# josehu07/summerset

Measured on AMD Instinct MI355X. Metric: committed_slots_per_sec, higher is better.
Workload: dtype u64; 1 GPU; MultiPaxos lock-step, 65536 groups/GPU x 5 replicas, S=32 new slots/group/tick, heartbeat every 4 ticks, 10% ack loss (<= 2 lost per slot), 59.53% of the groups per 4286 ticks with a leader timeout (9; groups_per_gpu=65536, replicas=5, slots_per_tick=32, window=512, layout=colocated

## Files before the change

### include/summerset_hip.h

```cpp
#ifndef SUMMERSET_HIP_H
#define SUMMERSET_HIP_H

#include <stddef.h>
#include <stdint.h>

#ifdef __cplusplus
extern "C" {
#endif

#define SMR_OK 0
#define SMR_ERR_ARG (-1)
#define SMR_ERR_DEVICE (-2)
#define SMR_ERR_STATE (-3)

#define SMR_NO_REPLICA 0xFFu
#define SMR_MAX_REPLICAS 8

enum { SMR_ST_NULL = 0, SMR_ST_PREPARING = 1, SMR_ST_ACCEPTING = 2, SMR_ST_COMMITTED = 3, SMR_ST_EXECUTED = 4 };

#define SMR_CTL_IDENTITY 0x00FAC688u

const char *smr_last_error(void);
int smr_device_count(void);
uint32_t smr_abi_version(void);
// ... 126 lines not shown

int smr_mp_ack_matrix(smr_mp_cluster *c, uint8_t rep, uint8_t **ack_dev, uint64_t *n_bytes);

typedef struct {
    uint32_t group, slot;
    uint64_t ballot;
    uint32_t peer;
    uint32_t reserved;
} smr_mp_ack;
int smr_mp_deliver_acks(smr_mp_cluster *c, uint8_t rep, const smr_mp_ack *acks_dev, uint64_t n, uint64_t *dropped_dev,
                        void *stream);
int smr_mp_deliver_acks_conn(smr_mp_cluster *c, uint8_t rep, const void *acks12_dev, uint64_t ack_cap, const uint64_t *conn_off_dev,
                             const uint32_t *conn_group_dev, const uint8_t *conn_peer_dev, const uint32_t *cnt_dev, uint32_t n_conn,
                             uint64_t *dropped_dev, void *stream);
int smr_mp_collect_acks(smr_mp_cluster *c, uint8_t rep, smr_mp_ack *out_dev, uint64_t cap, uint64_t *n_dev, void *stream);
int smr_mp_clear_acks(smr_mp_cluster *c, uint8_t rep, void *stream);

int smr_mp_debug_arena_view(smr_mp_cluster *c, void **base_dev, uint64_t *n_bytes);

int smr_mp_read_group_state(smr_mp_cluster *c, uint32_t group, uint8_t rep, smr_mp_group_state *out);

typedef struct {
    uint8_t *leader; uint64_t *bal_prep_sent, *bal_prepared, *bal_max_seen;
    uint32_t *start_slot, *log_len, *accept_bar, *commit_bar, *exec_bar, *snap_bar;
    uint32_t *peer_exec_bar;
    uint64_t *s_bal; uint8_t *s_status; uint32_t *s_reqs; uint64_t *s_vbal; uint32_t *s_vreqs;
    uint8_t *s_flags, *s_acks, *s_packs; uint64_t *s_pmax; uint32_t *s_ltrig, *s_lendp;
    uint8_t *s_src; uint32_t *s_rtrig, *s_rendp;
    uint8_t *overflow;
} smr_mp_dump_bufs;
int smr_mp_dump(smr_mp_cluster *c, uint8_t rep, const smr_mp_dump_bufs *host_bufs);
int smr_mp_dump_range(smr_mp_cluster *c, uint8_t rep, uint32_t g0, uint32_t n, const smr_mp_dump_bufs *host_bufs);

typedef struct smr_mp_snapshot smr_mp_snapshot;
typedef struct {
    uint64_t bytes;
    uint64_t n_slots, n_outbox;
    uint32_t n_groups, max_live, max_outbox;
    uint8_t population, commit_extra, live_mask, reserved;
} smr_mp_snapshot_info;
int smr_mp_snapshot_create(const smr_mp_cluster *like, smr_mp_snapshot **out);
void smr_mp_snapshot_destroy(smr_mp_snapshot *s);
int smr_mp_save_state(smr_mp_cluster *c, smr_mp_snapshot *s, void *stream);
int smr_mp_load_state(smr_mp_cluster *c, const smr_mp_snapshot *s, void *stream);
int smr_mp_snapshot_info_get(const smr_mp_snapshot *s, smr_mp_snapshot_info *out);
int64_t smr_mp_snapshot_export(const smr_mp_snapshot *s, uint8_t *host, uint64_t cap);
int smr_mp_snapshot_import(smr_mp_snapshot *s, const uint8_t *host, uint64_t len);

int smr_mp_counters(smr_mp_cluster *c, uint8_t rep, uint64_t out[3]);

int smr_mp_debug_generic_units(smr_mp_cluster *c, uint8_t rep, uint64_t *out);

int smr_mp_debug_folded_batches(smr_mp_cluster *c, uint8_t rep, uint64_t *out);

int smr_mp_straggler_stats(smr_mp_cluster *c, uint64_t out[2]);

int smr_mp_debug_stamps(smr_mp_cluster *c, uint64_t *out64);

int smr_mp_poll_commits(smr_mp_cluster *c, uint8_t rep, uint32_t *groups_host, uint32_t *slots_host,
                        uint64_t cap, uint64_t *n_out);

int smr_mp_profile_enable(smr_mp_cluster *c, int on);
int smr_mp_profile_read(smr_mp_cluster *c, int which, double *total_ms, uint64_t *launches);

typedef struct smr_raft_leader smr_raft_leader;

typedef struct {
    uint32_t n_groups;
    uint8_t population;
    uint8_t leader_id;
    uint8_t commit_extra;
    uint8_t reserved0;
    uint32_t window;
    uint64_t term;
} smr_raft_cfg;

int smr_raft_leader_create(const smr_raft_cfg *cfg, smr_raft_leader **out);
void smr_raft_leader_destroy(smr_raft_leader *l);
int smr_raft_leader_append(smr_raft_leader *l, const uint32_t *n_new_dev, void *stream);
int smr_raft_leader_handle_replies(smr_raft_leader *l, const uint64_t *reply_term_dev,
                                   const uint32_t *end_slot_dev, const uint64_t *conflict_term_dev,
                                   const uint32_t *conflict_slot_dev, const uint8_t *flags_dev,
                                   const uint32_t *order_dev, void *stream);
typedef struct {
    const uint32_t *n_new;
    const uint64_t *reply_term;
    const uint32_t *end_slot;
    const uint64_t *conflict_term;
    const uint32_t *conflict_slot;
    const uint8_t *flags;
    const uint32_t *order;
} smr_raft_tick;
int smr_raft_leader_run_ticks(smr_raft_leader *l, const smr_raft_tick *ticks, uint32_t n_ticks, void *stream);
typedef struct {
    uint8_t *role; uint64_t *curr_term; uint32_t *log_len, *last_commit, *last_snap;
    uint32_t *next_slot, *try_next_slot, *match_slot;
    uint64_t *entry_term;
    uint8_t *leader; uint32_t *start_slot;
} smr_raft_dump_bufs;
int smr_raft_leader_dump(smr_raft_leader *l, const smr_raft_dump_bufs *host_bufs);
int smr_raft_leader_total_commits(smr_raft_leader *l, uint64_t *out);

int smr_raft_craft_enable(smr_raft_leader *l, uint8_t fault_tolerance, uint8_t repeat_threshold);
int smr_raft_craft_bcast_heartbeats(smr_raft_leader *l, uint8_t *hb_flags_dev, uint32_t *prev_slot_dev, uint64_t *prev_term_dev,
                                    uint32_t *leader_commit_dev, uint32_t *last_snap_dev, void *stream);
int smr_raft_craft_switch_assignment_mode(smr_raft_leader *l, const uint8_t *to_full_dev, void *stream);
// ... 651 lines not shown
```

### summerset_amd/_lib.py

```python
import ctypes as C
import os

_HERE = os.path.dirname(os.path.abspath(__file__))
LIB_PATH = os.path.join(_HERE, "libsummerset_hip.so")

SMR_OK, SMR_ERR_ARG, SMR_ERR_DEVICE, SMR_ERR_STATE = 0, -1, -2, -3
SMR_NO_REPLICA = 0xFF
SMR_MAX_REPLICAS = 8
SMR_CTL_IDENTITY = 0x00FAC688


class SummersetError(RuntimeError):

    def __init__(self, code, msg):
        super().__init__("[%d] %s" % (code, msg))
        self.code = code
        self.msg = msg


class MpCfg(C.Structure):
    _fields_ = [("n_groups", C.c_uint32), ("population", C.c_uint8), ("commit_extra", C.c_uint8),
                ("straggler_ticks", C.c_uint8), ("reserved1", C.c_uint8), ("window", C.c_uint32),
                ("win_reserve", C.c_uint32), ("outbox_cap", C.c_uint32), ("commit_list_cap", C.c_uint32)]

# ... 190 lines not shown
    _fields_ = [("kind", C.c_uint8), ("has_voted", C.c_uint8), ("n_items", C.c_uint32), ("slot", C.c_uint64),
                ("ballot", C.c_uint64), ("trigger_slot", C.c_uint64), ("endprep_slot", C.c_uint64), ("voted_ballot", C.c_uint64),
                ("commit_bar", C.c_uint64), ("exec_bar", C.c_uint64), ("snap_bar", C.c_uint64)]


SYMBOLS = [
    ("smr_last_error", C.c_char_p, []),
    ("smr_device_count", _i, []),
    ("smr_abi_version", _u32, []),
    ("smr_rs_matrix", _i, [_i, _i, _vp]),
    ("smr_rs_shard_len", _u64, [_u64, _i]),
    ("smr_rs_encode", _i, [_vp, _u64, _u64, _u64, _i, _i, _vp, _u64, _u64, _vp]),
    ("smr_rs_encode_lut", _i, [_vp, _u64, _u64, _u64, _i, _i, _vp, _u64, _u64, _vp]),
    ("smr_rs_from_data_encode", _i, [_vp, _u64, _u64, _u64, _i, _i, _vp, _u64, _vp]),
    ("smr_rs_from_data_encode_fanout", _i, [_vp, _u64, _u64, _u64, _i, _i, _vp, _u64, _vp, _u64, _u64, _u32, _vp]),
    ("smr_rs_from_data_encode_stores", _i, [_vp, _u64, _u64, _u64, _i, _i, _vp, _u64, _u64, _vp]),
    ("smr_rs_from_data_encode_scatter", _i, [_vp, _u64, _u64, _u64, _i, _i, _vp, _u64, _vp, _u64, _vp]),
    ("smr_rs_reconstruct", _i, [_vp, _u64, _u64, _u64, _u64, _i, _i, _u32, _i, _vp]),
    ("smr_rs_verify", _i, [_vp, _u64, _u64, _u64, _u64, _i, _i, _vp, _vp]),
    ("smr_mp_cluster_create", _i, [C.POINTER(MpCfg), C.POINTER(_vp)]),
    ("smr_mp_cluster_destroy", None, [_vp]),
    ("smr_mp_preset_leader", _i, [_vp, _u8]),
    ("smr_mp_tick", _i, [_vp, _vp, _vp, _vp, _vp, _vp, _u32, _vp, _i, _vp]),
    ("smr_mp_run_ticks", _i, [_vp, C.POINTER(MpTickIn), _u32, _vp]),
    ("smr_mp_set_live", _i, [_vp, _u32]),
    ("smr_mp_set_role_rotation", _i, [_vp, _i]),
    ("smr_mp_image_bytes", C.c_int64, [_vp, _i, _u32, _u32]),
    ("smr_mp_image_pack", _i, [_vp, _i, _u8, _u8, _vp, _u64, _u32, _u32, _vp]),
    ("smr_mp_image_unpack", _i, [_vp, _i, _u8, _u8, _vp, _u64, _u32, _u32, _vp]),
    ("smr_mp_image_plan_create", _i, [C.POINTER(MpImageOp), _u32, _u32, _u32, C.POINTER(_vp)]),
    ("smr_mp_image_plan_destroy", None, [_vp]),
    ("smr_mp_image_plan_run", _i, [_vp, _i, _vp]),
    ("smr_mp_round_local", _i, [_vp, _vp, _vp, _vp, _vp, _vp, _u32, _vp]),
    ("smr_mp_round_deliver", _i, [_vp, _vp]),
    ("smr_mp_round_replies", _i, [_vp, _vp, _i, _vp]),
    ("smr_mp_round_heartbeat", _i, [_vp, _vp]),
    ("smr_mp_end_tick", _i, [_vp]),
    ("smr_mp_spread_create", _i, [_vp, _u32, _vp, _vp, _vp]),
    ("smr_mp_spread_destroy", None, [_vp]),
    ("smr_mp_spread_segment", _i, [_vp, _i, _vp, _i, _vp]),
    ("smr_mp_spread_set_concurrent", _i, [_vp, _i]),
    ("smr_mp_spread_abort_tick", _i, [_vp]),
    ("smr_mp_ack_matrix", _i, [_vp, _u8, C.POINTER(_vp), C.POINTER(_u64)]),
    ("smr_mp_deliver_acks", _i, [_vp, _u8, _vp, _u64, _vp, _vp]),
    ("smr_mp_deliver_acks_conn", _i, [_vp, _u8, _vp, _u64, _vp, _vp, _vp, _vp, _u32, _vp, _vp]),
    ("smr_mp_collect_acks", _i, [_vp, _u8, _vp, _u64, _vp, _vp]),
    ("smr_mp_clear_acks", _i, [_vp, _u8, _vp]),
    ("smr_mp_read_group_state", _i, [_vp, _u32, _u8, C.POINTER(MpGroupState)]),
    ("smr_mp_dump", _i, [_vp, _u8, C.POINTER(MpDumpBufs)]),
    ("smr_mp_dump_range", _i, [_vp, C.c_uint8, _u32, _u32, C.POINTER(MpDumpBufs)]),
    ("smr_mp_counters", _i, [_vp, _u8, C.POINTER(_u64 * 3)]),
    ("smr_mp_debug_generic_units", _i, [_vp, _u8, C.POINTER(_u64)]),
    ("smr_mp_debug_folded_batches", _i, [_vp, _u8, C.POINTER(_u64)]),
    ("smr_mp_debug_stamps", _i, [_vp, _vp]),
    ("smr_comm_unique_id", _i, [_vp, _u64]),
    ("smr_comm_init_rank", _i, [_vp, _u64, _u32, _u32, C.POINTER(_vp)]),
    ("smr_comm_destroy", None, [_vp]),
    ("smr_comm_exchange", _i, [_vp, _vp, C.POINTER(_u64), _vp, C.POINTER(_u64), _u32, _vp]),
    ("smr_comm_all_reduce_u64", _i, [_vp, _vp, _u64, _i, _vp]),
    ("smr_comm_info", _i, [_vp, C.POINTER(_u64 * 5)]),
    ("smr_mp_spread_bind_comm", _i, [_vp, _vp, C.POINTER(_vp * 3), C.POINTER(_u64), C.POINTER(_vp * 3), C.POINTER(_u64), _u32]),
    ("smr_mp_spread_tick", _i, [_vp, _vp, _i, _vp]),
    ("smr_mp_straggler_stats", _i, [_vp, C.POINTER(_u64 * 2)]),
    ("smr_mp_poll_commits", _i, [_vp, _u8, _vp, _vp, _u64, C.POINTER(_u64)]),
    ("smr_mp_debug_arena_view", _i, [_vp, C.POINTER(_vp), C.POINTER(_u64)]),
    ("smr_mp_snapshot_create", _i, [_vp, C.POINTER(_vp)]),
    ("smr_mp_snapshot_destroy", None, [_vp]),
    ("smr_mp_save_state", _i, [_vp, _vp, _vp]),
    ("smr_mp_load_state", _i, [_vp, _vp, _vp]),
    ("smr_mp_snapshot_info_get", _i, [_vp, C.POINTER(MpSnapshotInfo)]),
    ("smr_mp_snapshot_export", C.c_int64, [_vp, _vp, _u64]),
    ("smr_mp_snapshot_import", _i, [_vp, _vp, _u64]),
    ("smr_mp_profile_enable", _i, [_vp, _i]),
    ("smr_mp_profile_read", _i, [_vp, _i, C.POINTER(C.c_double), C.POINTER(_u64)]),
    ("smr_raft_leader_create", _i, [C.POINTER(RaftCfg), C.POINTER(_vp)]),
    ("smr_raft_leader_destroy", None, [_vp]),
    ("smr_raft_leader_append", _i, [_vp, _vp, _vp]),
    ("smr_raft_leader_handle_replies", _i, [_vp, _vp, _vp, _vp, _vp, _vp, _vp, _vp]),
    ("smr_raft_leader_handle_wire_replies", _i, [_vp, _vp, _u64, _vp, _vp, _u32, _vp, _vp, _u64, _vp, _vp, _vp, _vp]),
    ("smr_raft_leader_run_ticks", _i, [_vp, _vp, _u32, _vp]),
    ("smr_raft_leader_dump", _i, [_vp, C.POINTER(RaftDumpBufs)]),
    ("smr_raft_leader_total_commits", _i, [_vp, C.POINTER(_u64)]),
    ("smr_raft_replica_preset", _i, [_vp, _u8, _u8, _u64, _u8]),
    ("smr_raft_replica_handle_append_entries", _i, [_vp, C.POINTER(RaftAppendEntries), C.POINTER(RaftAppendReply), _vp]),
    ("smr_raft_replica_become_candidate", _i, [_vp, _vp, _vp, _vp, _vp, _vp, _vp]),
    ("smr_raft_replica_handle_request_vote", _i, [_vp, _vp, _vp, _vp, _vp, _vp, _vp, _vp, _vp]),
    ("smr_raft_replica_handle_vote_replies", _i, [_vp, _vp, _vp, _vp, _vp, _vp, _vp]),
    ("smr_raft_replica_dump_votes", _i, [_vp, _vp, _vp, _vp, _vp]),
    ("smr_raft_leader_append_emit", _i, [_vp, _vp, _vp, _vp]),
    ("smr_raft_leader_gather_entries", _i, [_vp, _vp, C.POINTER(RaftAppendEntries), _vp]),
    ("smr_raft_cluster_replicate", _i, [_vp, _u32, C.POINTER(_vp), C.POINTER(_vp), C.POINTER(RaftAppendEntries), C.POINTER(RaftAppendReply), _vp]),
    ("smr_raft_cluster_tick", _i, [_vp, _vp, _vp, _u32, C.POINTER(_vp), C.POINTER(_vp), C.POINTER(RaftAppendEntries), C.POINTER(RaftAppendReply), _vp, _vp, _vp, _vp, _vp, _vp, _vp]),
    ("smr_raft_craft_enable", _i, [_vp, _u8, _u8]),
    ("smr_raft_craft_bcast_heartbeats", _i, [_vp, _vp, _vp, _vp, _vp, _vp, _vp]),
    ("smr_raft_craft_switch_assignment_mode", _i, [_vp, _vp, _vp]),
    ("smr_raft_craft_assignment", _i, [_vp, _vp, _vp, _vp]),
    ("smr_raft_craft_dump", _i, [_vp, _vp, _vp, _vp, _vp, _vp]),
    ("smr_raft_craft_handle_reconstruct", _i, [_vp, _vp, _vp, _vp, _u32, _vp, _vp, _vp, _vp]),
    ("smr_raft_craft_dump_masks", _i, [_vp, _vp, _vp]),
    ("smr_raft_ring_guard_hits", _i, [_vp, C.POINTER(_u64)]),
    ("smr_raft_snapshot_create", _i, [_vp, C.POINTER(_vp)]),
    ("smr_raft_snapshot_destroy", None, [_vp]),
    ("smr_raft_save_state", _i, [_vp, _vp, _vp]),
    ("smr_raft_load_state", _i, [_vp, _vp, _vp]),
    ("smr_raft_snapshot_info_get", _i, [_vp, C.POINTER(RaftSnapshotInfo)]),
    ("smr_raft_snapshot_export", C.c_int64, [_vp, _vp, _u64]),
# ... 243 lines not shown
```

### summerset_amd/csrc/mp_engine.hip

```cpp
#include <stdlib.h>
#include <string.h>

#include <algorithm>
#include <functional>
#include <vector>

#include "mp_device.h"
#include "smr_common.h"
#include "mp_snapshot.h"

#ifdef SMR_BULK_PRIO
#define SMR_RAISE_PRIO() __builtin_amdgcn_s_setprio(SMR_BULK_PRIO)
#else
#define SMR_RAISE_PRIO() ((void)0)
#endif

namespace smr {

__device__ __forceinline__ void flush_counters(const Lane &L, bool active) {
    unsigned int c[4] = {active ? L.n_commit : 0u, active ? L.n_redirect : 0u, active ? L.n_reject : 0u,
                         active ? L.n_generic : 0u};
    const bool any = (c[0] | c[1] | c[2] | c[3]) != 0;
    for (unsigned long long todo = __ballot(any); todo;) {
        const uint32_t rep = __shfl(L.me, __ffsll((long long)todo) - 1);
// ... 1180 lines not shown
    uint32_t g;
    const bool active = pick_group(P, side, g);
    r4_body(P, par, g, active, pick_replica(P, side, g));
}

#ifndef STRAG_MINW
#define STRAG_MINW 1
#endif
#ifndef STRAG_K
#define STRAG_K 1
#endif
__global__ __launch_bounds__(512, STRAG_MINW) void mp_straggler_tick(const MpParams *__restrict__ Pp, int par, int lpar,
                                                          const uint8_t *__restrict__ timeout_rep,
                                                          const uint8_t *__restrict__ timeout_src,
                                                          const uint8_t *__restrict__ req_target,
                                                          const uint32_t *__restrict__ req_cnt,
                                                          const uint32_t *__restrict__ req_val, uint32_t S,
                                                          const uint32_t *__restrict__ ackctl, int do_heartbeat) {
    const MpParams &P = *Pp;
    const uint32_t w = threadIdx.x >> 6, lane = threadIdx.x & 63;
    uint32_t n = P.slow_n[lpar];
    if (n > P.slow_cap) n = P.slow_cap;
    for (uint32_t idx0 = blockIdx.x; idx0 < n; idx0 += gridDim.x * STRAG_K) {
        const uint32_t idx = idx0 + lane * gridDim.x;
        const bool mine = w < P.R && lane < STRAG_K && idx < n;
        const uint32_t g = mine ? P.slow_list[idx] : P.G;
        const uint32_t r = w < P.R ? w : 0;
        if (timeout_rep || req_target)
            r1_body(P, par, timeout_rep, timeout_src, req_target, req_cnt, req_val, S, g, mine && !P.overflow[g], r);
        __syncthreads();
        r2_body<0>(P, par, g, mine && !P.overflow[g], r);
        __syncthreads();
        r3_body(P, par, ackctl, do_heartbeat, g, mine && !P.overflow[g], r);
        __syncthreads();
        if (do_heartbeat) {
            r4_body(P, par, g, mine && !P.overflow[g], r);
            __syncthreads();
        }
    }
}

#ifndef STRAG_BATCH_K
#define STRAG_BATCH_K 6
#endif
#ifndef STRAG_COOP
#define STRAG_COOP true
#endif
#ifndef STRAG_BATCH_BLOCKS
#define STRAG_BATCH_BLOCKS 192
#endif
#ifndef STRAG_BATCH_MINW
#define STRAG_BATCH_MINW STRAG_MINW
#endif
__global__ __launch_bounds__(512, STRAG_BATCH_MINW) void mp_straggler_batch(const MpParams *__restrict__ Pp, int lpar, const MpTickBatch B) {
    const MpParams &P = *Pp;
    const uint32_t w = threadIdx.x >> 6, lane = threadIdx.x & 63;
    uint32_t n = P.slow_n[lpar];
    if (n > P.slow_cap) n = P.slow_cap;
#ifdef STRAG_PACK
    for (uint32_t idx0 = blockIdx.x * STRAG_PACK; idx0 < n; idx0 += gridDim.x * STRAG_PACK) {
        const uint32_t idx = idx0 + lane;
        const bool mine = w < P.R && lane < STRAG_PACK && idx < n;
#else
    for (uint32_t idx0 = blockIdx.x; idx0 < n; idx0 += gridDim.x * STRAG_BATCH_K) {
        const uint32_t idx = idx0 + lane * gridDim.x;
        const bool mine = w < P.R && lane < STRAG_BATCH_K && idx < n;
#endif
        const uint32_t g = mine ? P.slow_list[idx] : P.G;
        const uint32_t r = w < P.R ? w : 0;
        for (uint32_t t = 0; t < B.n; t++) {
            const MpTickIn &in = B.t[t];
            const int par = B.par0 ^ (int)(t & 1u);
            if (in.timeout_rep || in.req_target)
                r1_body(P, par, in.timeout_rep, in.timeout_src, in.req_target, in.req_cnt, in.req_val, in.S, g, mine && !P.overflow[g], r, STRAG_COOP);
            __syncthreads();
            r2_body<0>(P, par, g, mine && !P.overflow[g], r, STRAG_COOP);
            __syncthreads();
            r3_body(P, par, in.ackctl, in.heartbeat, g, mine && !P.overflow[g], r, STRAG_COOP);
            __syncthreads();
            if (in.heartbeat) {
                r4_body(P, par, g, mine && !P.overflow[g], r);
                __syncthreads();
            }
        }
    }
}

__global__ __launch_bounds__(256) void mp_mark_batch(const MpParams *__restrict__ Pp, int lpar, const MpTickBatch B, uint32_t ttl) {
    const MpParams &P = *Pp;
    const uint32_t g = blockIdx.x * 256 + threadIdx.x;
    if (g == 0) P.slow_n[lpar ^ 1] = 0;
    if (g >= P.G) return;
    mark_role(P, g);
    uint32_t t = P.slow_ttl[g];
    bool any = false;
    for (uint32_t k = 0; k < B.n; k++) {
        const uint8_t *tr = B.t[k].timeout_rep;
        if (tr && tr[g] != NO_REP) t = ttl;
        if (t > 0) { any = true; t--; }
    }
    uint8_t s = 0;
    if (any) {
        const uint32_t idx = atomicAdd(&P.slow_n[lpar], 1u);
        if (idx < P.slow_cap) { P.slow_list[idx] = g; s = 1; }
    }
    P.slow_ttl[g] = (uint8_t)t;
    if (P.slow[g] != s) P.slow[g] = s;
}

__device__ __forceinline__ void fused_r1(const MpParams *Pp, int par, const uint8_t *timeout_rep, const uint8_t *timeout_src,
                                      const uint8_t *req_target, const uint32_t *req_cnt, const uint32_t *req_val, uint32_t S,
                                      uint32_t g, uint32_t r) {
    r1_body(*Pp, par, timeout_rep, timeout_src, req_target, req_cnt, req_val, S, g, g < Pp->G && !Pp->overflow[g], r);
}
__device__ __forceinline__ void fused_r2(const MpParams *Pp, int par, uint32_t g, uint32_t r) {
    r2_body<0>(*Pp, par, g, g < Pp->G && !Pp->overflow[g], r);
}
template <int NR>
__device__ __forceinline__ void fused_tally(const MpParams *Pp, int par, const uint32_t *ackctl, int publish_hb, uint8_t *sh_fl,
                                         uint32_t *sh_mk) {
    quorum_tally_block<NR>(*Pp, par, ackctl, publish_hb, sh_fl, sh_mk, 0u);
}
__device__ __forceinline__ void fused_r3(const MpParams *Pp, int par, const uint32_t *ackctl, int publish_hb, uint32_t g, uint32_t r) {
    r3_body(*Pp, par, ackctl, publish_hb, g, g < Pp->G && !Pp->overflow[g], r);
}
__device__ __forceinline__ void fused_r4(const MpParams *Pp, int par, uint32_t g, uint32_t r) {
    r4_body(*Pp, par, g, g < Pp->G && !Pp->overflow[g], r);
}

#ifndef FUSED_MINW
#define FUSED_MINW 2
#endif
template <int NR, int NW>
__global__ __launch_bounds__(NW * 64, FUSED_MINW) void mp_ticks_fused(const MpParams *__restrict__ Pp, const MpTickBatch B) {
    __shared__ uint8_t sh_fl[64 * 64];
    __shared__ uint32_t sh_mk[64 * 64];
    const uint32_t w = threadIdx.x >> 6, lane = threadIdx.x & 63;
// ... 330 lines not shown
    const bool active = pick_group(P, 0, g);
    r2_body<0>(P, M.par[blockIdx.z], g, active, pick_replica(P, 0, g));
}
template <int NR>
__global__ __launch_bounds__(256, TALLY_MINW) void mp_quorum_tally_multi(const MpMulti M, int publish_hb) {
    __shared__ uint8_t sh_fl[64 * 64];
    __shared__ uint32_t sh_mk[64 * 64];
    const MpParams &P = *M.p[blockIdx.z];
    if (blockIdx.x * 64u >= P.G) return;
    quorum_tally_block<NR>(P, M.par[blockIdx.z], M.in[blockIdx.z].ackctl, publish_hb, sh_fl, sh_mk, M.hint[blockIdx.z]);
}
__global__ __launch_bounds__(256) void mp_round_replies_multi(const MpMulti M, int publish_hb) {
    const MpParams &P = *M.p[blockIdx.z];
    if (blockIdx.x * blockDim.x >= P.G || !((P.live >> blockIdx.y) & 1u)) return;
    {
        const uint32_t ntile = (P.G + 63) / 64, tpb = blockDim.x >> 6, t0 = blockIdx.x * tpb;
        uint32_t any = 0;
        for (uint32_t k = 0; k < tpb; k++) any |= (t0 + k < ntile) ? P.r3_need[(size_t)blockIdx.y * ntile + t0 + k] : 0u;
        if (!any) return;
    }
    uint32_t g;
    const bool active = pick_group(P, 0, g);
    r3_body(P, M.par[blockIdx.z], M.in[blockIdx.z].ackctl, publish_hb, g, active, pick_replica(P, 0, g));
}
__global__ __launch_bounds__(256) void mp_round_heartbeat_multi(const MpMulti M) {
    const MpParams &P = *M.p[blockIdx.z];
    if (blockIdx.x * blockDim.x >= P.G || !((P.live >> blockIdx.y) & 1u)) return;
    uint32_t g;
    const bool active = pick_group(P, 0, g);
    r4_body(P, M.par[blockIdx.z], g, active, pick_replica(P, 0, g));
}

}

using namespace smr;

struct smr_mp_cluster {
    smr_mp_cfg cfg;
    MpParams hp;
    MpParams *dp = nullptr;
    Arena arena;
    uint32_t pcap = 0;
    int par = 0;
    int lpar = 0;
    uint32_t ttl = 0;
    hipStream_t side = nullptr;
    hipEvent_t ev_fork = nullptr, ev_join = nullptr;
    bool forked = false, marked = false, side_on = false, side_fused = false;
    uint32_t side_live = 0;
    uint32_t quiet_ticks = 0;
    bool always_defer = false;
    bool no_split_r2 = true;
    bool split_r2 = false;
    MpNextLocal next_local = MpNextLocal{nullptr, nullptr, nullptr, nullptr, 0u};
    bool fold_r1 = false;
    bool defer_rest = false;
    bool rest_pending = false;
    int rest_par = 0;
    const uint32_t *rest_ackctl = nullptr;
    uint32_t lead_hint = 0;
    bool spread_open = false;
    bool profile = false;
    std::vector<ProfEv> evs;
    double prof_ms[5] = {0, 0, 0, 0, 0};
    uint64_t prof_n[5] = {0, 0, 0, 0, 0};
};

namespace smr {

#ifndef SMR_SLOW_CAP
#define SMR_SLOW_CAP 1024
#endif
constexpr uint32_t SLOW_CAP = SMR_SLOW_CAP;

static bool is_pow2(uint32_t x) { return x && !(x & (x - 1)); }

template <typename T> static void carve(Arena &a, T *&p, size_t n, bool dry) {
    size_t off = a.reserve(n * sizeof(T));
    if (!dry) p = a.at<T>(off);
}

static void layout(smr_mp_cluster *c, bool dry) {
    Arena &a = c->arena;
    a.used = 0;
    const size_t G = c->cfg.n_groups, W = c->cfg.window, R = c->cfg.population, cap = c->cfg.outbox_cap,
                 pcap = c->pcap;
    const size_t Gp = (G + 63) / 64 * 64;
    MpParams &P = c->hp;
    carve(a, P.overflow, G, dry);
    carve(a, P.dbg, 64, dry);
    carve(a, P.r3_need, R * ((G + 63) / 64), dry);
    carve(a, P.r2_need, R * ((G + 63) / 64), dry); carve(a, P.r2_res, R * G, dry);
    carve(a, P.slow, G, dry); carve(a, P.slow_ttl, G, dry); carve(a, P.role_rot, G, dry);
    carve(a, P.r1_done, G, dry);
    carve(a, P.slow_list, (size_t)SLOW_CAP, dry); carve(a, P.slow_n, 2, dry);
    for (size_t r = 0; r < R; r++) {
        MpRep &v = P.rep[r];
        carve(a, v.leader, G, dry);
        carve(a, v.bal_prep_sent, G, dry); carve(a, v.bal_prepared, G, dry); carve(a, v.bal_max_seen, G, dry);
        carve(a, v.start_slot, G, dry); carve(a, v.log_len, G, dry); carve(a, v.accept_bar, G, dry);
        carve(a, v.commit_bar, G, dry); carve(a, v.exec_bar, G, dry); carve(a, v.snap_bar, G, dry);
        carve(a, v.null_lb, G, dry);
        carve(a, v.bal_lo, G, dry);
        carve(a, v.peer_exec_bar, R * G, dry);
        carve(a, v.s_bal, W * Gp, dry); carve(a, v.s_val, W * Gp, dry); carve(a, v.s_meta, W * Gp, dry);
        carve(a, v.s_vbal, W * Gp, dry); carve(a, v.s_vval, W * Gp, dry); carve(a, v.s_pmax, W * Gp, dry);
// ... 82 lines not shown
}

}

extern "C" {

int smr_mp_cluster_create(const smr_mp_cfg *cfg, smr_mp_cluster **out) {
    if (!cfg || !out) return fail(SMR_ERR_ARG, "mp: null argument");
    if (cfg->n_groups == 0) return fail(SMR_ERR_ARG, "mp: n_groups is zero");
    if (cfg->population < 3 || cfg->population > SMR_MAX_REPLICAS)
        return fail(SMR_ERR_ARG, "mp: population must be in 3..8");
    if (!is_pow2(cfg->window) || cfg->window < 8 || cfg->window > (1u << 20))
        return fail(SMR_ERR_ARG, "mp: window must be a power of two in 8..2^20");
    if (cfg->win_reserve >= cfg->window) return fail(SMR_ERR_ARG, "mp: win_reserve >= window");
    if (cfg->outbox_cap < 4) return fail(SMR_ERR_ARG, "mp: outbox_cap < 4");
    uint32_t quorum = cfg->population / 2 + 1;
    if (cfg->commit_extra > cfg->population - quorum)
        return fail(SMR_ERR_ARG, "mp: commit_extra (fault_tolerance) exceeds population - majority");
    smr_mp_cluster *c = new smr_mp_cluster();
    c->cfg = *cfg;
    c->pcap = cfg->window;
    memset(&c->hp, 0, sizeof(c->hp));
    layout(c, true);
    c->arena.size = c->arena.used + 256;
    hipError_t e = hipMalloc((void **)&c->arena.base, c->arena.size);
    if (e != hipSuccess) {
        delete c;
        return fail(SMR_ERR_DEVICE, std::string("mp: hipMalloc of engine state: ") + hipGetErrorString(e));
    }
    layout(c, false);
    MpParams &P = c->hp;
    P.G = cfg->n_groups; P.W = cfg->window; P.Wmask = cfg->window - 1; P.cap = cfg->outbox_cap;
    P.pcap = c->pcap; P.win_reserve = cfg->win_reserve; P.clist_cap = cfg->commit_list_cap;
    P.R = cfg->population; P.quorum = quorum; P.thresh = quorum + cfg->commit_extra; P.rspaxos = 0;
    P.slow_cap = SLOW_CAP;
    P.live = (1u << cfg->population) - 1u;
    if (!stride_ok(P)) {
        (void)hipFree(c->arena.base);
        delete c;
        return fail(SMR_ERR_DEVICE, "mp: replica arrays are not equally spaced in the arena");
    }
    e = hipMemset(c->arena.base, 0, c->arena.size);
    for (uint32_t r = 0; e == hipSuccess && r < P.R; r++) e = hipMemset(P.rep[r].leader, 0xFF, P.G);
    if (e == hipSuccess) e = hipMalloc((void **)&c->dp, sizeof(MpParams));
    if (e == hipSuccess) e = hipMemcpy(c->dp, &c->hp, sizeof(MpParams), hipMemcpyHostToDevice);
    if (e != hipSuccess) {
        (void)hipFree(c->arena.base);
        if (c->dp) (void)hipFree(c->dp);
        delete c;
        return fail(SMR_ERR_DEVICE, std::string("mp: init: ") + hipGetErrorString(e));
    }
    c->ttl = cfg->straggler_ticks == SMR_STRAGGLER_OFF ? 0u : cfg->straggler_ticks;
    c->no_split_r2 = getenv("SMR_MP_SPLIT_R2") == nullptr;
    c->always_defer = getenv("SMR_MP_ALWAYS_DEFER_REST") != nullptr;
    c->fold_r1 = getenv("SMR_MP_FOLD_R1") != nullptr;
    if (c->ttl) {
        e = hipStreamCreateWithFlags(&c->side, hipStreamNonBlocking);
        if (e == hipSuccess) e = hipEventCreateWithFlags(&c->ev_fork, hipEventDisableTiming);
        if (e == hipSuccess) e = hipEventCreateWithFlags(&c->ev_join, hipEventDisableTiming);
        if (e != hipSuccess) {
            smr_mp_cluster_destroy(c);
            return fail(SMR_ERR_DEVICE, std::string("mp: side stream: ") + hipGetErrorString(e));
        }
    }
    *out = c;
    return SMR_OK;
}

void smr_mp_cluster_destroy(smr_mp_cluster *c) {
    if (!c) return;
    (void)hipDeviceSynchronize();
    if (c->ev_fork) (void)hipEventDestroy(c->ev_fork);
    if (c->ev_join) (void)hipEventDestroy(c->ev_join);
    if (c->side) (void)hipStreamDestroy(c->side);
    for (auto &e : c->evs) { (void)hipEventDestroy(e.a); (void)hipEventDestroy(e.b); }
    if (c->dp) (void)hipFree(c->dp);
    if (c->arena.base) (void)hipFree(c->arena.base);
    delete c;
}

int smr_mp_preset_leader(smr_mp_cluster *c, uint8_t rep) {
    if (!c || rep >= c->cfg.population) return fail(SMR_ERR_ARG, "mp: bad replica id");
    const uint32_t G = c->cfg.n_groups;
    std::vector<uint64_t> b(G, (1ull << 8) | (uint64_t)(rep + 1));
    for (uint32_t r = 0; r < c->cfg.population; r++) {
        MpRep &v = c->hp.rep[r];
        SMR_HIP_TRY(hipMemset(v.leader, rep, G));
        SMR_HIP_TRY(hipMemcpy(v.bal_max_seen, b.data(), G * 8, hipMemcpyHostToDevice));
        if (r == rep) {
            SMR_HIP_TRY(hipMemcpy(v.bal_prep_sent, b.data(), G * 8, hipMemcpyHostToDevice));
            SMR_HIP_TRY(hipMemcpy(v.bal_prepared, b.data(), G * 8, hipMemcpyHostToDevice));
        }
    }
    c->lead_hint = rep;
    return SMR_OK;
}

int smr_mp_round_local(smr_mp_cluster *c, const uint8_t *timeout_rep_dev, const uint8_t *timeout_src_dev,
                       const uint8_t *req_target_dev, const uint32_t *req_cnt_dev, const uint32_t *req_val_dev,
                       uint32_t S, void *stream) {
    if (!c) return fail(SMR_ERR_ARG, "mp: null cluster");
    if (timeout_rep_dev && !timeout_src_dev) return fail(SMR_ERR_ARG, "mp: timeout_rep without timeout_src");
    if (req_target_dev && (!req_cnt_dev || !req_val_dev)) return fail(SMR_ERR_ARG, "mp: incomplete request arrays");
    hipStream_t st = (hipStream_t)stream;
    int rc = ensure_marked(c, timeout_rep_dev, st); if (rc) return rc;
    if (!timeout_rep_dev && !req_target_dev) {
// ... 127 lines not shown
                           timeout_rep_dev, timeout_src_dev, req_target_dev, req_cnt_dev, req_val_dev, S, ackctl_dev,
                           do_heartbeat);
        SMR_HIP_TRY(hipGetLastError());
        c->side_fused = true;
    }
    rc = smr_mp_round_local(c, timeout_rep_dev, timeout_src_dev, req_target_dev, req_cnt_dev, req_val_dev, S, stream);
    if (!rc) rc = smr_mp_round_deliver(c, stream);
    if (!rc) rc = smr_mp_round_replies(c, ackctl_dev, do_heartbeat, stream);
    if (!rc && do_heartbeat) rc = smr_mp_round_heartbeat(c, stream);
    c->side_fused = false;
    const int rj = join_side(c, st, own);
    if (rc) return rc;
    if (rj) return rj;
    return smr_mp_end_tick(c);
}

int smr_mp_run_ticks(smr_mp_cluster *c, const smr_mp_tick_in *ticks, uint32_t n, void *stream) {
    if (!c || (n && !ticks)) return fail(SMR_ERR_ARG, "mp: null argument");
    if (c->hp.live != (1u << c->cfg.population) - 1u) return fail(SMR_ERR_STATE, "mp: run_ticks needs every replica live (co-located layout)");
    if (c->forked || c->marked) return fail(SMR_ERR_STATE, "mp: run_ticks inside an open tick");
    hipStream_t st = (hipStream_t)stream;
    for (uint32_t i = 0; i < n; i++) {
        const smr_mp_tick_in &x = ticks[i];
        if (x.timeout_rep_dev && !x.timeout_src_dev) return fail(SMR_ERR_ARG, "mp: timeout_rep without timeout_src");
        if (x.req_target_dev && (!x.req_cnt_dev || !x.req_val_dev)) return fail(SMR_ERR_ARG, "mp: incomplete request arrays");
    }
    const uint32_t R = c->cfg.population;
    const dim3 grid((c->cfg.n_groups + 63) / 64);
    for (uint32_t i0 = 0; i0 < n; i0 += MP_FUSED_MAXT) {
        MpTickBatch b;
        memset(&b, 0, sizeof(b));
        b.n = n - i0 < MP_FUSED_MAXT ? n - i0 : MP_FUSED_MAXT;
        b.par0 = c->par;
        for (uint32_t k = 0; k < b.n; k++) {
            const smr_mp_tick_in &x = ticks[i0 + k];
            b.t[k] = MpTickIn{x.timeout_rep_dev, x.timeout_src_dev, x.req_target_dev, x.req_cnt_dev, x.req_val_dev, x.ackctl_dev,
                              x.S, x.do_heartbeat ? 1 : 0};
        }
        if (!c->ttl) {
            if (R <= 5) hipLaunchKernelGGL((mp_ticks_fused<5, 5>), grid, dim3(5 * 64), 0, st, c->dp, b);
            else hipLaunchKernelGGL((mp_ticks_fused<MAXR, MAXR>), grid, dim3(MAXR * 64), 0, st, c->dp, b);
            SMR_HIP_TRY(hipGetLastError());
            c->par ^= (int)(b.n & 1u);
            continue;
        }
        bool any_to = false;
        for (uint32_t k = 0; k < b.n; k++) any_to = any_to || ticks[i0 + k].timeout_rep_dev != nullptr;
        c->quiet_ticks = any_to ? 0u : c->quiet_ticks + b.n;
        const bool quiet = c->quiet_ticks >= 2u * MP_FUSED_MAXT + c->ttl;
        hipLaunchKernelGGL(mp_mark_batch, dim3((c->cfg.n_groups + 255) / 256), dim3(256), 0, st, c->dp, c->lpar, b, c->ttl);
        SMR_HIP_TRY(hipGetLastError());
        SMR_HIP_TRY(hipEventRecord(c->ev_fork, st));
        SMR_HIP_TRY(hipStreamWaitEvent(c->side, c->ev_fork, 0));
        hipLaunchKernelGGL(mp_straggler_batch, dim3(STRAG_BATCH_BLOCKS), dim3(R <= 5 ? 320 : 512), 0, c->side, c->dp, c->lpar, b);
        SMR_HIP_TRY(hipGetLastError());
        c->marked = c->side_on = c->forked = c->side_fused = true;
        c->split_r2 = !quiet && !c->no_split_r2;
        int rc = SMR_OK;
        for (uint32_t k = 0; k < b.n && !rc; k++) {
            const smr_mp_tick_in &x = ticks[i0 + k];
            rc = smr_mp_round_local(c, x.timeout_rep_dev, x.timeout_src_dev, x.req_target_dev, x.req_cnt_dev, x.req_val_dev, x.S, stream);
            if (!rc) rc = smr_mp_round_deliver(c, stream);
            c->defer_rest = k + 1 < b.n && (quiet || c->always_defer);
            if (k + 1 < b.n && !x.do_heartbeat && c->fold_r1 && ticks[i0 + k + 1].req_target_dev) {
                const smr_mp_tick_in &y = ticks[i0 + k + 1];
                c->next_local = MpNextLocal{y.timeout_rep_dev, y.req_target_dev, y.req_cnt_dev, y.req_val_dev, y.S};
            }
            if (!rc) rc = smr_mp_round_replies(c, x.ackctl_dev, x.do_heartbeat ? 1 : 0, stream);
            c->next_local = MpNextLocal{nullptr, nullptr, nullptr, nullptr, 0u};
            c->defer_rest = false;
            if (!rc && x.do_heartbeat) rc = smr_mp_round_heartbeat(c, stream);
            c->par ^= 1;
        }
        if (c->rest_pending) {
            c->rest_pending = false;
            hipLaunchKernelGGL(mp_round_replies, mp_grid(c), dim3(MP_BLOCK), 0, st, c->dp, c->rest_par, c->rest_ackctl, 0, 0);
        }
        c->marked = c->side_on = c->forked = c->side_fused = false;
        c->split_r2 = false;
        hipError_t e1 = hipEventRecord(c->ev_join, c->side);
        hipError_t e2 = hipStreamWaitEvent(st, c->ev_join, 0);
        c->lpar ^= 1;
        if (rc) return rc;
        SMR_HIP_TRY(e1);
        SMR_HIP_TRY(e2);
    }
    return SMR_OK;
}

int smr_mp_set_role_rotation(smr_mp_cluster *c, int on) {
    if (!c) return fail(SMR_ERR_ARG, "mp: null cluster");
    const uint32_t all = (1u << c->cfg.population) - 1u;
    if (on && c->hp.live != all) return fail(SMR_ERR_STATE, "mp: role rotation needs every replica on this device");
    if (on && !c->ttl) return fail(SMR_ERR_STATE, "mp: role rotation rides on the straggler mark pass (straggler_ticks > 0)");
    SMR_HIP_TRY(hipDeviceSynchronize());
    c->hp.rot_on = on ? 1u : 0u;
    SMR_HIP_TRY(hipMemset(c->hp.role_rot, 0, c->cfg.n_groups));
    SMR_HIP_TRY(hipMemcpy(c->dp, &c->hp, sizeof(MpParams), hipMemcpyHostToDevice));
    return SMR_OK;
}

int smr_mp_set_live(smr_mp_cluster *c, uint32_t live_mask) {
    if (!c) return fail(SMR_ERR_ARG, "mp: null cluster");
    const uint32_t all = (1u << c->cfg.population) - 1u;
    if ((live_mask & ~all) != 0) return fail(SMR_ERR_ARG, "mp: live mask names a replica beyond the population");
    if (c->ttl && live_mask != all) return fail(SMR_ERR_STATE, "mp: the spread layout and the straggler side stream exclude each other");
    if (c->hp.rot_on && live_mask != all) return fail(SMR_ERR_STATE, "mp: the spread layout and role rotation exclude each other");
// ... 247 lines not shown
            hb->s_bal[o] = k.bal; hb->s_status[o] = k.status; hb->s_reqs[o] = k.reqs;
            hb->s_vbal[o] = k.vbal; hb->s_vreqs[o] = k.vreqs;
            hb->s_flags[o] = k.flags; hb->s_acks[o] = k.acks; hb->s_packs[o] = k.packs;
            hb->s_pmax[o] = k.pmax; hb->s_ltrig[o] = k.ltrig; hb->s_lendp[o] = k.lendp;
            hb->s_src[o] = k.src; hb->s_rtrig[o] = k.rtrig; hb->s_rendp[o] = k.rendp;
        }
    }
    return SMR_OK;
}

int smr_mp_dump(smr_mp_cluster *c, uint8_t rep, const smr_mp_dump_bufs *hb) {
    if (!c) return fail(SMR_ERR_ARG, "mp: bad argument");
    return smr_mp_dump_range(c, rep, 0, c->cfg.n_groups, hb);
}

int smr_mp_counters(smr_mp_cluster *c, uint8_t rep, uint64_t out[3]) {
    if (!c || !out || rep >= c->cfg.population) return fail(SMR_ERR_ARG, "mp: bad argument");
    SMR_HIP_TRY(hipDeviceSynchronize());
    unsigned long long h[4];
    SMR_HIP_TRY(ctr_read((const unsigned long long *)c->hp.rep[rep].counters, 4, h));
    out[0] = h[0]; out[1] = h[1]; out[2] = h[2];
    return SMR_OK;
}

int smr_mp_straggler_stats(smr_mp_cluster *c, uint64_t out[2]) {
    if (!c || !out) return fail(SMR_ERR_ARG, "mp: bad argument");
    out[0] = c->ttl ? (uint64_t)SLOW_CAP : 0u; out[1] = 0;
    if (!c->ttl) return SMR_OK;
    SMR_HIP_TRY(hipDeviceSynchronize());
    uint32_t n[2];
    SMR_HIP_TRY(hipMemcpy(n, c->hp.slow_n, 8, hipMemcpyDeviceToHost));
    out[1] = n[c->lpar ^ 1];
    return SMR_OK;
}

int smr_mp_debug_generic_units(smr_mp_cluster *c, uint8_t rep, uint64_t *out) {
    if (!c || !out || rep >= c->cfg.population) return fail(SMR_ERR_ARG, "mp: bad argument");
    SMR_HIP_TRY(hipDeviceSynchronize());
    unsigned long long h[4];
    SMR_HIP_TRY(ctr_read((const unsigned long long *)c->hp.rep[rep].counters, 4, h));
    *out = h[3];
    return SMR_OK;
}

int smr_mp_debug_folded_batches(smr_mp_cluster *c, uint8_t rep, uint64_t *out) {
    if (!c || !out || rep >= c->cfg.population) return fail(SMR_ERR_ARG, "mp: bad argument");
    SMR_HIP_TRY(hipDeviceSynchronize());
    unsigned long long h[5];
    SMR_HIP_TRY(ctr_read((const unsigned long long *)c->hp.rep[rep].counters, 5, h));
    *out = h[4];
    return SMR_OK;
}

int smr_mp_debug_stamps(smr_mp_cluster *c, uint64_t *out64) {
    if (!c || !out64) return fail(SMR_ERR_ARG, "mp: bad argument");
    SMR_HIP_TRY(hipDeviceSynchronize());
    SMR_HIP_TRY(hipMemcpy(out64, c->hp.dbg, 64 * 8, hipMemcpyDeviceToHost));
    return SMR_OK;
}

int smr_mp_poll_commits(smr_mp_cluster *c, uint8_t rep, uint32_t *groups_host, uint32_t *slots_host, uint64_t cap,
                        uint64_t *n_out) {
    if (!c || rep >= c->cfg.population || !n_out) return fail(SMR_ERR_ARG, "mp: bad argument");
    if (c->cfg.commit_list_cap == 0) return fail(SMR_ERR_STATE, "mp: cluster was created without a commit list");
    SMR_HIP_TRY(hipDeviceSynchronize());
    const MpRep &v = c->hp.rep[rep];
    unsigned int n = 0;
    SMR_HIP_TRY(hipMemcpy(&n, v.clist_n, 4, hipMemcpyDeviceToHost));
    *n_out = n;
    uint64_t take = n;
    if (take > c->cfg.commit_list_cap) take = c->cfg.commit_list_cap;
    if (take > cap) take = cap;
    if (take && groups_host && slots_host) {
        std::vector<unsigned long long> tmp(take);
        SMR_HIP_TRY(hipMemcpy(tmp.data(), v.clist, take * 8, hipMemcpyDeviceToHost));
        for (uint64_t i = 0; i < take; i++) {
            groups_host[i] = (uint32_t)(tmp[i] >> 32);
            slots_host[i] = (uint32_t)tmp[i];
        }
    }
    SMR_HIP_TRY(hipMemset(v.clist_n, 0, 4));
    return SMR_OK;
}

int smr_mp_profile_enable(smr_mp_cluster *c, int on) {
    if (!c) return fail(SMR_ERR_ARG, "mp: null cluster");
    c->profile = on != 0;
    return SMR_OK;
}

int smr_mp_profile_read(smr_mp_cluster *c, int which, double *total_ms, uint64_t *launches) {
    if (!c || which < 0 || which > 4) return fail(SMR_ERR_ARG, "mp: bad argument");
    if (!c->evs.empty()) {
        SMR_HIP_TRY(hipDeviceSynchronize());
        for (auto &e : c->evs) {
            float ms = 0;
            SMR_HIP_TRY(hipEventElapsedTime(&ms, e.a, e.b));
            c->prof_ms[e.which] += ms;
            c->prof_n[e.which]++;
            (void)hipEventDestroy(e.a); (void)hipEventDestroy(e.b);
        }
        c->evs.clear();
    }
    if (total_ms) *total_ms = c->prof_ms[which];
    if (launches) *launches = c->prof_n[which];
    return SMR_OK;
// ... 416 lines not shown
```

### summerset_amd/multipaxos.py

```python
import ctypes as C

import numpy as np

from . import _lib
from .snapshot import DeviceSnapshot
from ._lib import MpCfg, MpDumpBufs, MpGroupState, MpTickIn, SummersetError, check, stream_ptr

_DUMP_T = {"leader": np.uint8, "bal_prep_sent": np.uint64, "bal_prepared": np.uint64, "bal_max_seen": np.uint64,
           "s_bal": np.uint64, "s_status": np.uint8, "s_reqs": np.uint32, "s_vbal": np.uint64,
           "s_vreqs": np.uint32, "s_flags": np.uint8, "s_acks": np.uint8, "s_packs": np.uint8,
           "s_pmax": np.uint64, "s_ltrig": np.uint32, "s_lendp": np.uint32, "s_src": np.uint8,
           "s_rtrig": np.uint32, "s_rendp": np.uint32, "overflow": np.uint8}


ACK_DTYPE = np.dtype([("group", "<u4"), ("slot", "<u4"), ("ballot", "<u8"), ("peer", "<u4"), ("reserved", "<u4")])


def _ptr(t):
    return None if t is None else t.data_ptr()


class MpSnapshot(DeviceSnapshot):
    _STEM, _INFO = "smr_mp_snapshot", _lib.MpSnapshotInfo

# ... 85 lines not shown
        off, grp, peer = ing.conn
        check(self._L.smr_mp_deliver_acks_conn(self._h, rep, _ptr(ing.acks), ing.ack_cap, _ptr(off), _ptr(grp), _ptr(peer), _ptr(ing.cnt), ing.n_conn,
                                               _ptr(dropped), stream_ptr(stream)))

    def clear_acks(self, rep, stream=None):
        check(self._L.smr_mp_clear_acks(self._h, rep, stream_ptr(stream)))

    def read_group_state(self, group, rep):
        st = MpGroupState()
        check(self._L.smr_mp_read_group_state(self._h, group, rep, C.byref(st)))
        return st

    def replica_log_view(self, rep):
        from ._lib import QreadLog
        view = QreadLog()
        check(self._L.smr_mp_replica_log_view(self._h, rep, C.byref(view)))
        return view

    def dump(self, rep, g0=0, n=None):
        W, R = self.W, self.R
        G = self.G - g0 if n is None else int(n)
        out, bufs = {}, MpDumpBufs()
        for name in _lib.MP_DUMP_FIELDS:
            t = _DUMP_T.get(name, np.uint32)
            shape = (R, G) if name == "peer_exec_bar" else ((W, G) if name.startswith("s_") else (G,))
            out[name] = np.zeros(shape, t)
            setattr(bufs, name, out[name].ctypes.data_as(C.c_void_p))
        check(self._L.smr_mp_dump_range(self._h, rep, int(g0), G, C.byref(bufs)))
        return out

    def save_state(self, snap=None, stream=None):
        snap = MpSnapshot(self) if snap is None else snap
        check(self._L.smr_mp_save_state(self._h, snap._h, stream_ptr(stream)))
        return snap

    def load_state(self, snap, stream=None):
        check(self._L.smr_mp_load_state(self._h, snap._h, stream_ptr(stream)))

    def counters(self, rep):
        arr = (C.c_uint64 * 3)()
        check(self._L.smr_mp_counters(self._h, rep, C.byref(arr)))
        return {"commits": int(arr[0]), "redirects": int(arr[1]), "rejects": int(arr[2])}

    def debug_generic_units(self, rep):
        n = C.c_uint64()
        check(self._L.smr_mp_debug_generic_units(self._h, rep, C.byref(n)))
        return int(n.value)

    def debug_folded_batches(self, rep):
        n = C.c_uint64()
        check(self._L.smr_mp_debug_folded_batches(self._h, rep, C.byref(n)))
        return int(n.value)

    def straggler_stats(self):
        arr = (C.c_uint64 * 2)()
        check(self._L.smr_mp_straggler_stats(self._h, C.byref(arr)))
        return int(arr[0]), int(arr[1])

    def poll_commits(self, rep, cap=None):
        cap = self.commit_list_cap if cap is None else cap
        g = np.zeros(cap, np.uint32)
        s = np.zeros(cap, np.uint32)
        n = C.c_uint64()
        check(self._L.smr_mp_poll_commits(self._h, rep, g.ctypes.data_as(C.c_void_p),
                                          s.ctypes.data_as(C.c_void_p), cap, C.byref(n)))
        if n.value > cap:
            raise SummersetError(_lib.SMR_ERR_STATE, "commit list overflowed: %d > %d" % (n.value, cap))
        return g[:n.value].copy(), s[:n.value].copy()

    def profile_enable(self, on=True):
        check(self._L.smr_mp_profile_enable(self._h, int(on)))

    def profile_read(self, which):
        ms, n = C.c_double(), C.c_uint64()
        check(self._L.smr_mp_profile_read(self._h, which, C.byref(ms), C.byref(n)))
        return ms.value, n.value
```

Measured before the change: 22.97 billion slots/s.

## Add steady-state fast path for straggler groups in side batch kernel

Adds a per-group steady-tick fast path to the straggler batch kernel. It checks across replicas (through shared memory) that a group has a stable leader, no timeout, no pending outbox and matching log lengths and ballots. If so, it appends new requests, writes follower acks directly, and processes replies in one pass instead of the full r1/r2/r3 round sequence. Groups that fail the check fall back to the generic rounds. This adds per-group serial checks, extra syncthreads and counter atomics, and risks correctness if the fast path diverges from the generic protocol.

```diff
diff --git a/include/summerset_hip.h b/include/summerset_hip.h
--- a/include/summerset_hip.h
+++ b/include/summerset_hip.h
@@ -202,6 +202,8 @@
 int smr_mp_debug_generic_units(smr_mp_cluster *c, uint8_t rep, uint64_t *out);
 
 int smr_mp_debug_folded_batches(smr_mp_cluster *c, uint8_t rep, uint64_t *out);
+
+int smr_mp_debug_side_steps(smr_mp_cluster *c, uint64_t out[2]);
 
 int smr_mp_straggler_stats(smr_mp_cluster *c, uint64_t out[2]);
 
diff --git a/summerset_amd/_lib.py b/summerset_amd/_lib.py
--- a/summerset_amd/_lib.py
+++ b/summerset_amd/_lib.py
@@ -266,6 +266,7 @@
     ("smr_mp_counters", _i, [_vp, _u8, C.POINTER(_u64 * 3)]),
     ("smr_mp_debug_generic_units", _i, [_vp, _u8, C.POINTER(_u64)]),
     ("smr_mp_debug_folded_batches", _i, [_vp, _u8, C.POINTER(_u64)]),
+    ("smr_mp_debug_side_steps", _i, [_vp, C.POINTER(_u64 * 2)]),
     ("smr_mp_debug_stamps", _i, [_vp, _vp]),
     ("smr_comm_unique_id", _i, [_vp, _u64]),
     ("smr_comm_init_rank", _i, [_vp, _u64, _u32, _u32, C.POINTER(_vp)]),
diff --git a/summerset_amd/csrc/mp_engine.hip b/summerset_amd/csrc/mp_engine.hip
--- a/summerset_amd/csrc/mp_engine.hip
+++ b/summerset_amd/csrc/mp_engine.hip
@@ -1256,37 +1256,136 @@
 #ifndef STRAG_BATCH_MINW
 #define STRAG_BATCH_MINW STRAG_MINW
 #endif
-__global__ __launch_bounds__(512, STRAG_BATCH_MINW) void mp_straggler_batch(const MpParams *__restrict__ Pp, int lpar, const MpTickBatch B) {
+#ifdef STRAG_PACK
+#define SIDE_K STRAG_PACK
+#else
+#define SIDE_K STRAG_BATCH_K
+#endif
+static_assert(SIDE_K >= 1 && SIDE_K <= 32, "listed groups per block: a bit each in the tick's `done` mask");
+constexpr uint32_t SIDE_REC = 6;
+
+__device__ __forceinline__ bool side_steady_tick(const MpParams &P, int par, const MpTickIn &in, const uint32_t g, const uint32_t w,
+                                                 uint32_t *__restrict__ sh) {
+    const bool rep = w < P.R;
+    Lane J(P, rep ? w : 0, g, par);
+    J.set_uniform();
+    const RepView &v = J.v;
+    const uint32_t to = in.timeout_rep ? in.timeout_rep[g] : NO_REP;
+    const uint32_t tgt = in.req_target ? in.req_target[g] : NO_REP;
+    uint32_t n = in.req_target ? in.req_cnt[g] : 0u;
+    const uint32_t tok = (in.req_target && J.cl < in.S) ? in.req_val[(size_t)J.cl * P.G + g] : 0u;
+    const uint32_t frozen = P.overflow[g], r1d = P.r1_done[g];
+    uint32_t c_par = 0, pr_mine = 0;
+    if (rep) {
+        J.load();
+        c_par = v.ob_cnt(par)[g];
+        pr_mine = v.pr_cnt()[g];
+    }
+    if (n > in.S) n = in.S;
+    if (tgt >= P.R) n = 0;
+    const bool lead = rep && J.is_leader();
+    bool ok = rep && to == NO_REP && !frozen && r1d == 0 && c_par == 0 && J.leader < P.R && (n == 0 || tgt == J.leader) && n <= 64u;
+    if (lead)
+        ok = ok && J.bpd != 0 && J.bpd == J.bms && P.thresh > 1 && J.nlb >= J.len && J.abar == J.len && n <= P.cap &&
+             (J.len - J.start) + n + P.win_reserve <= P.W;
+    else
+        ok = ok && J.abar == J.len && (J.len - J.start) + n <= P.W;
+    if (rep && J.wr) {
+        const uint64_t bal = lead ? J.bpd : J.bms;
+        uint32_t *const my = sh + w * SIDE_REC;
+        my[0] = J.leader; my[1] = ok ? 1u : 0u; my[2] = J.len; my[3] = (uint32_t)bal; my[4] = (uint32_t)(bal >> 32);
+    }
+    __syncthreads();
+    const uint32_t l = sh[0];
+    bool all = l < P.R;
+    if (all) {
+        const uint32_t *const lr = sh + l * SIDE_REC;
+        for (uint32_t q = 0; q < P.R; q++) {
+            const uint32_t *const qr = sh + q * SIDE_REC;
+            all = all && qr[1] != 0 && qr[0] == l && qr[2] == lr[2] && qr[3] == lr[3] && qr[4] == lr[4];
+        }
+    }
+    if (!all) return false;
+    if (rep) {
+        if (lead) {
+            if (n) {
+                if (par == 0) { J.obn0 = 0; J.obl0 = true; } else { J.obn1 = 0; J.obl1 = true; }
+                (void)r1_coop_append(J, par, in.req_val, n);
+            }
+        } else {
+            if (pr_mine && J.wr) v.pr_cnt()[g] = 0;
+            if (n) {
+                const RepView snd{P.rep[0], (size_t)l * P.rep_stride};
+                const uint32_t r = J.me, k = J.cl;
+                if (k < n) {
+                    v.s_val()[tix(P.W, (J.len + k) & P.Wmask, g)] = tok;
+                    ACK_STORE(snd.ack(), k, 1);
+                }
+                if (J.wr) ack_bits_base(snd.ack(), P.cap, P.G)[tix(MAXR, r, g)] = ack_range_bits(0, n);
+                if (J.nlb == J.len) J.nlb = J.len + n;
+                if (J.brun == 0xFFFFFFFFu || J.brun > J.len) J.brun = J.len;
+                J.len += n; J.abar = J.len;
+            }
+        }
+    }
+    __syncthreads();
+    if (rep) {
+        if (lead && n) { if (P.R <= 5) r3_accept_replies<5>(J, in.ackctl, n); else r3_accept_replies<MAXR>(J, in.ackctl, n); }
+        if (in.heartbeat) r3_publish_hb(J);
+        J.store();
+        flush_job(J);
+    }
+    return true;
+}
+
+__global__ __launch_bounds__(512, STRAG_BATCH_MINW) void mp_straggler_batch(const MpParams *__restrict__ Pp, int lpar, const MpTickBatch B, int steady) {
+    __shared__ uint32_t sh_side[SIDE_K * MAXR * SIDE_REC];
     const MpParams &P = *Pp;
     const uint32_t w = threadIdx.x >> 6, lane = threadIdx.x & 63;
     uint32_t n = P.slow_n[lpar];
     if (n > P.slow_cap) n = P.slow_cap;
+    uint32_t n_step = 0, n_round = 0;
 #ifdef STRAG_PACK
     for (uint32_t idx0 = blockIdx.x * STRAG_PACK; idx0 < n; idx0 += gridDim.x * STRAG_PACK) {
         const uint32_t idx = idx0 + lane;
-        const bool mine = w < P.R && lane < STRAG_PACK && idx < n;
 #else
     for (uint32_t idx0 = blockIdx.x; idx0 < n; idx0 += gridDim.x * STRAG_BATCH_K) {
         const uint32_t idx = idx0 + lane * gridDim.x;
-        const bool mine = w < P.R && lane < STRAG_BATCH_K && idx < n;
 #endif
-        const uint32_t g = mine ? P.slow_list[idx] : P.G;
+        const bool listed = lane < SIDE_K && idx < n;
+        const bool mine = w < P.R && listed;
+        const uint32_t g = listed ? P.slow_list[idx] : P.G;
         const uint32_t r = w < P.R ? w : 0;
+        const uint32_t nk = (uint32_t)__popcll(__ballot(listed));
         for (uint32_t t = 0; t < B.n; t++) {
             const MpTickIn &in = B.t[t];
             const int par = B.par0 ^ (int)(t & 1u);
-            if (in.timeout_rep || in.req_target)
-                r1_body(P, par, in.timeout_rep, in.timeout_src, in.req_target, in.req_cnt, in.req_val, in.S, g, mine && !P.overflow[g], r, STRAG_COOP);
-            __syncthreads();
-            r2_body<0>(P, par, g, mine && !P.overflow[g], r, STRAG_COOP);
-            __syncthreads();
-            r3_body(P, par, in.ackctl, in.heartbeat, g, mine && !P.overflow[g], r, STRAG_COOP);
-            __syncthreads();
+            uint32_t done = 0;
+            if (steady)
+                for (uint32_t k = 0; k < nk; k++)
+                    if (side_steady_tick(P, par, in, __shfl(g, (int)k), w, sh_side + k * (MAXR * SIDE_REC))) done |= 1u << k;
+            n_step += (uint32_t)__popc(done); n_round += nk - (uint32_t)__popc(done);
+            if (done != (nk >= 32u ? ~0u : (1u << nk) - 1u)) {
+                const bool rest = mine && !((done >> (lane & 31u)) & 1u);
+                if (in.timeout_rep || in.req_target)
+                    r1_body(P, par, in.timeout_rep, in.timeout_src, in.req_target, in.req_cnt, in.req_val, in.S, g, rest && !P.overflow[g], r, STRAG_COOP);
+                __syncthreads();
+                r2_body<0>(P, par, g, rest && !P.overflow[g], r, STRAG_COOP);
+                __syncthreads();
+                r3_body(P, par, in.ackctl, in.heartbeat, g, rest && !P.overflow[g], r, STRAG_COOP);
+                __syncthreads();
+            } else if (in.heartbeat) {
+                __syncthreads();
+            }
             if (in.heartbeat) {
                 r4_body(P, par, g, mine && !P.overflow[g], r);
                 __syncthreads();
             }
         }
+    }
+    if (threadIdx.x == 0) {
+        if (n_step) ctr_add((unsigned long long *)P.rep[0].counters, 5, (unsigned long long)n_step);
+        if (n_round) ctr_add((unsigned long long *)P.rep[0].counters, 6, (unsigned long long)n_round);
     }
 }
 
@@ -1723,6 +1822,7 @@
     bool always_defer = false;
     bool no_split_r2 = true;
     bool split_r2 = false;
+    bool side_steady = true;
     MpNextLocal next_local = MpNextLocal{nullptr, nullptr, nullptr, nullptr, 0u};
     bool fold_r1 = false;
     bool defer_rest = false;
@@ -1911,6 +2011,7 @@
     }
     c->ttl = cfg->straggler_ticks == SMR_STRAGGLER_OFF ? 0u : cfg->straggler_ticks;
     c->no_split_r2 = getenv("SMR_MP_SPLIT_R2") == nullptr;
+    { const char *e_ = getenv("SMR_MP_SIDE_STEADY"); c->side_steady = !(e_ && e_[0] == '0' && e_[1] == 0); }
     c->always_defer = getenv("SMR_MP_ALWAYS_DEFER_REST") != nullptr;
     c->fold_r1 = getenv("SMR_MP_FOLD_R1") != nullptr;
     if (c->ttl) {
@@ -2144,7 +2245,7 @@
         SMR_HIP_TRY(hipGetLastError());
         SMR_HIP_TRY(hipEventRecord(c->ev_fork, st));
         SMR_HIP_TRY(hipStreamWaitEvent(c->side, c->ev_fork, 0));
-        hipLaunchKernelGGL(mp_straggler_batch, dim3(STRAG_BATCH_BLOCKS), dim3(R <= 5 ? 320 : 512), 0, c->side, c->dp, c->lpar, b);
+        hipLaunchKernelGGL(mp_straggler_batch, dim3(STRAG_BATCH_BLOCKS), dim3(R <= 5 ? 320 : 512), 0, c->side, c->dp, c->lpar, b, c->side_steady ? 1 : 0);
         SMR_HIP_TRY(hipGetLastError());
         c->marked = c->side_on = c->forked = c->side_fused = true;
         c->split_r2 = !quiet && !c->no_split_r2;
@@ -2498,6 +2599,15 @@
     return SMR_OK;
 }
 
+int smr_mp_debug_side_steps(smr_mp_cluster *c, uint64_t out[2]) {
+    if (!c || !out) return fail(SMR_ERR_ARG, "mp: bad argument");
+    SMR_HIP_TRY(hipDeviceSynchronize());
+    unsigned long long h[7];
+    SMR_HIP_TRY(ctr_read((const unsigned long long *)c->hp.rep[0].counters, 7, h));
+    out[0] = h[5]; out[1] = h[6];
+    return SMR_OK;
+}
+
 int smr_mp_debug_stamps(smr_mp_cluster *c, uint64_t *out64) {
     if (!c || !out64) return fail(SMR_ERR_ARG, "mp: bad argument");
     SMR_HIP_TRY(hipDeviceSynchronize());
diff --git a/summerset_amd/multipaxos.py b/summerset_amd/multipaxos.py
--- a/summerset_amd/multipaxos.py
+++ b/summerset_amd/multipaxos.py
@@ -161,6 +161,11 @@
         check(self._L.smr_mp_debug_folded_batches(self._h, rep, C.byref(n)))
         return int(n.value)
 
+    def debug_side_steps(self):
+        arr = (C.c_uint64 * 2)()
+        check(self._L.smr_mp_debug_side_steps(self._h, C.byref(arr)))
+        return int(arr[0]), int(arr[1])
+
     def straggler_stats(self):
         arr = (C.c_uint64 * 2)()
         check(self._L.smr_mp_straggler_stats(self._h, C.byref(arr)))
```

New measurement: 24.30 billion slots/s, median of 6. 5.8% higher.
